# ServiceFoundation/partisan

Measured on AMD Instinct MI355X. Metric: simulated node-rounds/sec (+ msgs/sec), 1M-node HyParView+Plumtree, higher is better.
Workload: dtype u32

## Files before the change

### partisan_amd/csrc/psim_consume.hip

```cpp
#include "psim_device.h"
#include "psim_kernels.h"
#include "psim_lite.h"
#include "psim_wave.h"

namespace psim {

#define ID_OF(e, n) (((uint32_t)(e) << 20) | (uint32_t)(n))
#define ID_E(id) ((id) >> 20)
#define ID_C(id) ((id)&0xFFFFFu)

constexpr int WAVES_PER_BLOCK = 4;
#ifndef PSIM_WAVES_PER_SIMD
#define PSIM_WAVES_PER_SIMD 4
#endif

#ifdef PSIM_STAMPS
__device__ unsigned long long g_stamps[32];
__device__ unsigned long long g_stamps_lite[32];
#define STAMP(w, k)                                                                  \
    do {                                                                             \
        uint64_t t_ = __builtin_amdgcn_s_memtime();                                  \
        if (lane_id() == 0) (w).stl[(k)] += t_ - (w).t_last;                         \
        (w).t_last = t_;                                                             \
    } while (0)
// ... 1819 lines not shown
    uint4* o = reinterpret_cast<uint4*>(a.rec_out + slot);
    o[0] = make_uint4(dst, me, tt, seq);
    o[1] = make_uint4(a0, a1, a2, 0u);
    if (!PSIM_SHORT_TAIL || ((tt >> 16) & 0xFFu)) {
        o[2] = make_uint4(X[0], X[1], X[2], X[3]);
        o[3] = make_uint4(X[4], X[5], X[6], X[7]);
    }
    a.okey[slot] = dst | (max_emit(tt & 0xFF) << KEY_DST_BITS);
    return dg;
}

DEV void block_append(bool go, const uint4& D, uint4* desc, uint32_t* cnt, uint32_t* wcnt) {
    const uint64_t m = ballot(go);
    const uint32_t wv = threadIdx.x >> 6;
    __syncthreads();
    if (lane_id() == 0) wcnt[wv] = popc(m);
    __syncthreads();
    if (threadIdx.x == 0) {
        uint32_t t = 0;
        for (uint32_t k = 0; k < (blockDim.x >> 6); k++) t += wcnt[k];
        wcnt[4] = t ? atomicAdd(cnt, t) : 0u;
    }
    __syncthreads();
    if (go) {
        uint32_t b0 = wcnt[4];
        for (uint32_t k = 0; k < wv; k++) b0 += wcnt[k];
        desc[b0 + popc(m & lt_mask())] = D;
    }
}

#ifndef PSIM_RELAY_WAVES
#define PSIM_RELAY_WAVES 5
#endif
#ifndef PSIM_RELAY_FJ
#define PSIM_RELAY_FJ 1
#endif
#ifndef PSIM_PTL_BIN
#define PSIM_PTL_BIN 1
#endif
#ifndef PSIM_LITE_BIN
#define PSIM_LITE_BIN 1
#endif
__global__ void __launch_bounds__(256, PSIM_RELAY_WAVES) k_relay(RoundArgs) {
    if (*kargs().ctl) return;
    if (blockIdx.x == 0 && threadIdx.x == 0) kargs().ktime[0] = __builtin_amdgcn_s_memrealtime();
    enum { R_PROC, R_DELIV, R_SHUF, R_FAIL, R_DIGEST, R_BOUND, R_DELIV_FJ, R_FJ, R_N };
    __shared__ unsigned long long sst[R_N];
    __shared__ uint32_t wc5[11][5];
    if (threadIdx.x < R_N) sst[threadIdx.x] = 0;
    __syncthreads();
    const uint32_t l = lane_id();
    const uint32_t na = *kargs().n_alist;
    const uint64_t two58 = 1ull << 58;
    unsigned long long v[R_N] = {};
    for (uint32_t base = blockIdx.x * blockDim.x; base < na; base += gridDim.x * blockDim.x) {
        KArgs& a = kargs();
        const uint32_t P = base + threadIdx.x;
        uint4 D = make_uint4(0, 0, 0, 0);
        bool heavy = false, to_pt = false, relay = false, maps = false, shuf = false, lite = false, bcast = false, term = false,
             extra = false;
        Hdr h;
        uint32_t ik = 0, oend = 0;
        uint4 act0 = make_uint4(0, 0, 0, 0), act1 = act0;
        uint32_t me_part = 0;
        uint32_t hvm = 0;
        uint8_t fl0 = 0;
        if (P < na) {
            D = a.desc[P];
            const uint32_t id = D.x, tf = D.z >> 28;
            ik = D.z & DESC_CNT_MASK;
            const size_t li = id - a.lo;
            h = a.hdr[li];
            oend = (uint32_t)a.obase[li + 1];
            const uint4* ar = reinterpret_cast<const uint4*>(a.act + li * PSIM_ACTIVE_CAP);
            act0 = ar[0];
            act1 = ar[1];
            me_part = a.part[id];
            fl0 = a.flags[id];
            uint32_t hvn = 0;
            hvm = 0;
            bool all_relay = true, all_shuf = true, term_out = false, fjn = false;
            bcast = false; term = false; extra = (tf & DESC_SHUFFLE) != 0;
            const uint32_t av[8] = {act0.x, act0.y, act0.z, act0.w, act1.x, act1.y, act1.z, act1.w};
            for (uint32_t j = 0; j < ik; j += 4) {
                uint2 T[4];
#pragma unroll
                for (int q = 0; q < 4; q++) {
                    const uint4 r4 = j + q < ik ? *reinterpret_cast<const uint4*>(a.rec_in + D.y + j + q)
                                                : make_uint4(0, 0, (uint32_t)PSIM_MSG_PT_BROADCAST, 0);
                    T[q] = make_uint2(r4.y, r4.z);
                }
#pragma unroll
                for (int q = 0; q < 4; q++) {
                    const uint32_t tt = T[q].y, type = tt & 0xFF;
                    bcast |= j + q < ik && type == PSIM_MSG_PT_BROADCAST;
                    if (type < PSIM_MSG_PT_BROADCAST || type >= PSIM_MSG_XBOT_OPTIMIZATION) {
                        hvn++;
                        hvm |= j + q < 32 ? 1u << (j + q) : 0u;
                        maps |= type <= PSIM_MSG_NEIGHBOR_ACCEPTED;
                        const uint32_t ttl = (tt >> 8) & 0xFF;
                        const bool relays = ttl > 0 && h.act_n > 1;
                        const bool fj = PSIM_RELAY_FJ && !a.xbot && type == PSIM_MSG_FORWARD_JOIN && ttl > 0 &&
                                        ttl != a.prwl && h.act_n >= 4;
                        fjn |= fj;
                        all_relay &= (type == PSIM_MSG_SHUFFLE && ttl > 0) || fj;
                        all_shuf &= type == PSIM_MSG_SHUFFLE || type == PSIM_MSG_SHUFFLE_REPLY;
                        term |= type == PSIM_MSG_SHUFFLE && !relays;
                        extra |= type == PSIM_MSG_SHUFFLE && relays;
                        if (type == PSIM_MSG_SHUFFLE && !relays) {
                            bool in = false;
#pragma unroll
                            for (int k = 0; k < 8; k++) in |= (uint32_t)k < h.act_n && av[k] == T[q].x;
                            term_out |= !in;
                        }
                    }
                }
            }
            const bool fresh = h.start_round == a.round;
            bool exits = false;
            if (a.crash_round) {
                uint32_t cv[PSIM_CONN_CAP] = {};
                if (h.conn_n) {
                    const uint4* cr = reinterpret_cast<const uint4*>(a.conn + li * PSIM_CONN_CAP);
                    const uint4 c0 = cr[0], c1 = cr[1];
                    cv[0] = c0.x; cv[1] = c0.y; cv[2] = c0.z; cv[3] = c0.w;
                    cv[4] = c1.x; cv[5] = c1.y; cv[6] = c1.z; cv[7] = c1.w;
                }
#pragma unroll
                for (int j = 0; j < 8; j++) {
                    bool down = false;
#pragma unroll
                    for (int k = 0; k < PSIM_CONN_CAP; k++) down |= (uint32_t)k < h.conn_n && cv[k] == (av[j] | PSIM_CONN_DOWN);
                    exits |= (uint32_t)j < h.act_n && av[j] != id && av[j] < a.n_nodes && !down &&
                             crashed_now(a, av[j]);
                }
#pragma unroll
                for (int k = 0; k < PSIM_CONN_CAP; k++)
                    exits |= (uint32_t)k < h.conn_n && !(cv[k] & PSIM_CONN_DOWN) && crashed_now(a, cv[k] & KEY_DST_MASK);
            }
            const bool cdown = h.conn_dn != 0 && (hvn > 0 || (tf & DESC_SHUFFLE));
            const bool xwork = a.xbot && (h.conn_cl || (D.z & DESC_XBOT_BIT));
            bool fj_ok = true;
            if (fjn && a.plumtree) {
                const uint4* pr = reinterpret_cast<const uint4*>(a.pt_all + li * PSIM_PT_MEMBERS_CAP);
                const uint4 p0 = pr[0], p1 = pr[1];
                const uint32_t pv[8] = {p0.x, p0.y, p0.z, p0.w, p1.x, p1.y, p1.z, p1.w};
                fj_ok = h.all_n == h.act_n;
#pragma unroll
                for (int j = 0; j < 8; j++) {
                    bool in = false;
#pragma unroll
                    for (int k = 0; k < 8; k++) in |= (uint32_t)k < h.all_n && pv[k] == av[j];
                    fj_ok &= (uint32_t)j >= h.act_n || in;
                }
            }
            heavy = exits || fresh || ((tf & DESC_PROMO) && h.act_n < a.min_active) ||
                    (hvn && !all_shuf && !(all_relay && fj_ok)) || term_out || cdown || xwork;
            lite = !heavy && hvn && !(all_relay && h.act_n > 1);
            shuf = !heavy && !lite && (tf & DESC_SHUFFLE);
            maps = maps || exits || (tf & DESC_PROMO) || h.conn_cl;
            relay = !heavy && !lite && hvn > 0;
            const bool pt_msgs = !fresh && ik > hvn, origin = (tf & DESC_ORIGIN) != 0;
            const bool lazy = (tf & DESC_LAZY) && h.out_n > 0;
            to_pt = a.plumtree && (pt_msgs || origin || lazy);
            if (!heavy && !lite && (relay || to_pt || shuf)) v[R_PROC]++;
        }
        uint32_t upm[4] = {NONE, NONE, NONE, NONE};
        if (P < na && (relay || lite)) {
            const uint32_t av[8] = {act0.x, act0.y, act0.z, act0.w, act1.x, act1.y, act1.z, act1.w};
            KArgs& a = kargs();
#pragma unroll
            for (int j = 0; j < 8; j += 2) {
                const uint32_t q0 = (uint32_t)j < h.act_n && av[j] < a.n_nodes ? av[j] : D.x;
                const uint32_t q1 = (uint32_t)j + 1 < h.act_n && av[j + 1] < a.n_nodes ? av[j + 1] : D.x;
                upm[j >> 1] = (uint32_t)a.upart[q0] | ((uint32_t)a.upart[q1] << 16);
            }
        }
        const bool origin_node = ((D.z >> 28) & DESC_ORIGIN) != 0;
        {
            const bool ptl = P < na && to_pt && !origin_node, lt = P < na && lite;
            const bool pe = ptl && (!a.ptl_split || (!heavy && !lite && !shuf)), pl = ptl && !pe;
            const bool pb = bcast || !PSIM_PTL_BIN;
            const bool lt0 = lt && !(extra && PSIM_LITE_BIN), lt1 = lt && extra && PSIM_LITE_BIN;
            const bool tb = term || !PSIM_LITE_BIN;
            const bool g[11] = {P < na && heavy, P < na && to_pt && origin_node, pe && pb,
                                P < na && shuf, lt0 && tb, pe && !pb, lt0 && !tb,
                                lt1 && tb, lt1 && !tb, pl && pb, pl && !pb};
            uint64_t m[11];
#pragma unroll
            for (int k = 0; k < 11; k++) m[k] = ballot(g[k]);
            const uint32_t wv = threadIdx.x >> 6, nwv = blockDim.x >> 6;
            __syncthreads();
            if (l == 0)
#pragma unroll
                for (int k = 0; k < 11; k++) wc5[k][wv] = popc(m[k]);
            __syncthreads();
            if (threadIdx.x < 11) {
                const uint32_t k = threadIdx.x;
                uint32_t t = 0;
                for (uint32_t j = 0; j < nwv; j++) t += wc5[k][j];
                uint32_t* cnt = k == 0 ? a.n_slow : k == 1 ? a.n_pt : k == 2 ? a.n_ptl : k == 3 ? a.n_shuf
                              : k == 4 ? a.n_lite : k == 5 ? a.n_ptl + 1 : k < 9 ? a.n_lite + (k - 5)
                              : a.n_ptl + (k - 7);
                wc5[k][4] = t ? atomicAdd(cnt, t) : 0u;
            }
            __syncthreads();
#pragma unroll
            for (int k = 0; k < 11; k++)
                if (g[k]) {
                    uint32_t b0 = wc5[k][4];
                    for (uint32_t j = 0; j < wv; j++) b0 += wc5[k][j];
                    const uint32_t at = b0 + popc(m[k] & lt_mask());
                    uint4* desc = k == 0 ? a.desc_slow : k == 1 ? a.desc_pt : k == 2 || k == 5 || k >= 9 ? a.desc_ptl
                                : k == 3 ? a.desc_shuf : a.desc_lite;
                    const uint32_t nl = a.n_local;
                    desc[k == 5 || k == 6 ? nl - 1 - at : k == 7 || k == 9 ? nl + at
                         : k == 8 || k == 10 ? 2 * nl - 1 - at : at] =
                        k == 0 && maps ? make_uint4(D.x, D.y, D.z | DESC_MAPS_BIT, D.w) : D;
                }
        }
        if (P < na && lite && !heavy) {
            uint32_t cm = 0;
#pragma unroll
            for (int j = 0; j < 8; j++)
                cm |= ((upm[j >> 1] >> (16 * (j & 1))) & 0xFFFFu) == me_part ? 1u << j : 0u;
            kargs().lite_cm[D.x - kargs().lo] = (uint8_t)cm;
        }
        if (P >= na || heavy || lite) continue;
        const uint32_t id = D.x;
        const size_t li = id - a.lo;
        const uint32_t A[8] = {act0.x, act0.y, act0.z, act0.w, act1.x, act1.y, act1.z, act1.w};
        uint64_t rng = h.rng;
        uint32_t seq = 0;
        const bool big = ik > 32;
        uint32_t rm = relay ? hvm : 0u;
        for (uint32_t jr = 0; relay && (big ? jr < ik : rm != 0); jr++) {
            if (!big) {
                jr = (uint32_t)__ffs(rm) - 1;
                rm &= rm - 1;
            }
            const Msg* rp = a.rec_in + D.y + jr;
            const uint32_t tt = rp->tt;
            if ((tt & 0xFF) >= PSIM_MSG_PT_BROADCAST) continue;
            const bool fj = (tt & 0xFF) == PSIM_MSG_FORWARD_JOIN;
            const uint32_t ttl = (tt >> 8) & 0xFF, nex = (tt >> 16) & 0xFF, src = rp->src;
            const uint32_t jq = fj ? rp->a0 : NONE, jpe = fj ? rp->a1 : 0u;
            v[fj ? R_DELIV_FJ : R_DELIV]++;
            uint32_t elig = 0;
#pragma unroll
            for (int j = 0; j < 8; j++)
                elig |= (j < h.act_n && A[j] != src && A[j] != id && A[j] != jq) ? (1u << j) : 0u;
            const uint32_t cnt = __popc(elig);
            if (cnt) {
                uint32_t k;
                for (;;) {
                    const uint64_t x = draw58_at(rng++, id, a.seed);
                    if (x < cnt) { k = (uint32_t)x; break; }
                    const uint32_t i = mod_small(x, cnt);
                    if (x - i <= two58 - cnt) { k = i; break; }
                }
                uint32_t e = elig;
                for (uint32_t j = 0; j < k; j++) e &= e - 1;
                const uint32_t jr_ = (uint32_t)__ffs(e) - 1;
                const uint32_t r = A[jr_];
                uint32_t up = 0;
#pragma unroll
                for (int j = 0; j < 8; j++)
                    if ((uint32_t)j == jr_) up = (upm[j >> 1] >> (16 * (j & 1))) & 0xFFFFu;
                if (r < a.n_nodes && up == me_part) {
                    rng++;
                    uint32_t X[8] = {};
                    if (!fj) {
                        const uint4* ex = reinterpret_cast<const uint4*>(rp->ex);
                        const uint4 e0 = ex[0], e1 = ex[1];
                        const uint32_t E[8] = {e0.x, e0.y, e0.z, e0.w, e1.x, e1.y, e1.z, e1.w};
#pragma unroll
                        for (int j = 0; j < 8; j++) X[j] = (uint32_t)j < nex ? E[j] : 0u;
                    }
                    v[R_DIGEST] += relay_emit(a, D.w + seq, r, id,
                                              fj ? PSIM_MSG_FORWARD_JOIN | ((ttl - 1) << 8)
                                                 : PSIM_MSG_SHUFFLE | ((ttl - 1) << 8) | (nex << 16),
                                              seq, fj ? jq : 0u, jpe, 0u, X);
                    seq++;
                    v[fj ? R_FJ : R_SHUF]++;
                } else {
                    v[R_FAIL]++;
                }
            }
        }
        if (rng != h.rng) a.hdr[li].rng = rng;
        a.ocnt[li] = seq;
        v[R_BOUND] += seq > oend - D.w ? 1u : 0u;
        if (!to_pt) {
            a.flags[id] = (uint8_t)((fl0 & (F_UP | F_CRASHED)) | (h.out_n ? F_LAZY : 0) |
                                    (min((uint32_t)h.out_n, 15u) << F_OUTN_SHIFT) |
                                    (h.act_n < a.min_active ? F_LOWACT : 0));
        }
    }
#pragma unroll
    for (int k = 0; k < R_N; k++)
        for (int o = 32; o > 0; o >>= 1) v[k] += __shfl_xor(v[k], o);
    if (l == 0)
        for (int k = 0; k < R_N; k++)
            if (v[k]) atomicAdd(&sst[k], v[k]);
    __syncthreads();
    uint64_t* row = kargs().stat_relay + (size_t)blockIdx.x * NST;
    for (uint32_t k = threadIdx.x; k < NST; k += blockDim.x)
        row[k] = k == ST_PROC ? sst[R_PROC] : k == ST_DELIV + PSIM_MSG_SHUFFLE ? sst[R_DELIV]
               : k == ST_EMIT + PSIM_MSG_SHUFFLE ? sst[R_SHUF] : k == ST_FAIL ? sst[R_FAIL]
               : k == ST_DELIV + PSIM_MSG_FORWARD_JOIN ? sst[R_DELIV_FJ] : k == ST_EMIT + PSIM_MSG_FORWARD_JOIN ? sst[R_FJ]
               : k == ST_DIGEST ? sst[R_DIGEST] : k == ST_BOUND ? sst[R_BOUND] : 0ull;
}

constexpr int SHUF_TOPK = PSIM_EXCHANGE_CAP - 1;

DEV void topk_insert(uint64_t (&K)[SHUF_TOPK], uint32_t (&E)[SHUF_TOPK], uint64_t key, uint32_t e) {
    uint64_t ck = key;
    uint32_t ce = e;
#pragma unroll
    for (int i = 0; i < SHUF_TOPK; i++) {
        const bool lt = ck < K[i] || (ck == K[i] && ce < E[i]);
        const uint64_t tk = lt ? K[i] : ck;
        const uint32_t te = lt ? E[i] : ce;
        K[i] = lt ? ck : K[i];
        E[i] = lt ? ce : E[i];
        ck = tk;
        ce = te;
    }
}

enum { S_SHUF, S_FAIL, S_DIGEST, S_BOUND, S_N };
DEV void shuf_blocks(const uint32_t bid, const uint32_t nblk, unsigned long long* const sst) {
    if (*kargs().ctl) return;
    if (threadIdx.x < S_N) sst[threadIdx.x] = 0;
    __syncthreads();
    const uint32_t l = lane_id();
    const uint32_t ns = *kargs().n_shuf;
    const uint64_t two58 = 1ull << 58;
    unsigned long long v[S_N] = {};
    for (uint32_t P = bid * blockDim.x + threadIdx.x; P < ns; P += nblk * blockDim.x) {
        KArgs& a = kargs();
        const uint4 D = a.desc_shuf[P];
        const uint32_t id = D.x;
        const size_t li = id - a.lo;
        const uint64_t rng0 = a.hdr[li].rng;
        const uint32_t cnts = reinterpret_cast<const uint32_t*>(a.hdr + li)[9];
        const uint32_t act_n = cnts & 0xFF, pas_n = (cnts >> 8) & 0xFF;
        const uint4* ar = reinterpret_cast<const uint4*>(a.act + li * PSIM_ACTIVE_CAP);
        const uint4 a0 = ar[0], a1 = ar[1];
        const uint32_t A[8] = {a0.x, a0.y, a0.z, a0.w, a1.x, a1.y, a1.z, a1.w};
        uint32_t seq = a.ocnt[li];
        const uint32_t oend = (uint32_t)a.obase[li + 1];
        const uint32_t me_part = a.part[id];
        uint64_t rng = rng0;
        uint64_t K[SHUF_TOPK];
        uint32_t E[SHUF_TOPK];
#pragma unroll
// ... 762 lines not shown
```

### partisan_amd/csrc/psim_engine.hip

```cpp
#include <hip/hip_runtime.h>
#include <rccl/rccl.h>

#include <algorithm>
#include <chrono>
#include <cstdio>
#include <cstdlib>
#include <cstring>
#include <new>
#include <set>
#include <vector>

#include "psim_comm.h"
#include "psim_device.h"
#include "psim_kernels.h"
#include "psim_wave.h"

using namespace psim;

namespace {

constexpr int BLK = 256;
constexpr uint32_t PREP_BLK = 1024;
#ifndef PSIM_PREP_NPT
#define PSIM_PREP_NPT 4
// ... 1827 lines not shown
        release();
        p = nb.p; n = nb.n;
        return PSIM_OK;
    }
    int alloc(size_t want) {
        static const bool trace = getenv("PSIM_TRACE_GROW") != nullptr;
        if (trace && want >= (1u << 20)) std::fprintf(stderr, "psim: alloc %zu x %zu B\n", want, sizeof(T));
        if (hipMalloc(&p, std::max<size_t>(want, 1) * sizeof(T)) != hipSuccess) return PSIM_ENOMEM;
        n = want;
        if (hipMemset(p, 0, std::max<size_t>(want, 1) * sizeof(T)) != hipSuccess) return PSIM_EDEVICE;
        return PSIM_OK;
    }
    int alloc_on(size_t want, hipStream_t st) {
        if (hipMalloc(&p, std::max<size_t>(want, 1) * sizeof(T)) != hipSuccess) return PSIM_ENOMEM;
        n = want;
        if (hipMemsetAsync(p, 0, std::max<size_t>(want, 1) * sizeof(T), st) != hipSuccess) return PSIM_EDEVICE;
        return PSIM_OK;
    }
    void release() { if (p) (void)hipFree(p); p = nullptr; n = 0; }
};

template <typename T>
struct TmpBuf : DBuf<T> {
    TmpBuf() = default;
    TmpBuf(const TmpBuf&) = delete;
    TmpBuf& operator=(const TmpBuf&) = delete;
    ~TmpBuf() { this->release(); }
};

enum Kern { KT_EVENTS, KT_PREPARE, KT_CONSUME, KT_SCAN, KT_COMPACT, KT_SORT, KT_EXCHANGE, KT_GATHER,
            KT_STATS, KT_HOST_EXPORT, KT_HOST_IMPORT, KT_N };
const char* kKernName[KT_N] = {"events", "prepare", "consume", "scan", "compact", "sort",
                               "exchange", "gather", "stats", "k_host_export", "k_host_import"};

inline uint32_t grid_for(uint64_t n) { return (uint32_t)std::max<uint64_t>(1, (n + BLK - 1) / BLK); }

int bits_for(uint64_t n) {
    int b = 1;
    while (b < 32 && (1ull << b) < n) b++;
    return b;
}

constexpr uint64_t RESERVE_PER_NODE = 24;
constexpr uint64_t RCAP_PER_NODE = 4;
constexpr uint64_t RCAP_RESERVE = 8;
constexpr double RCAP_FREE_FRAC = 0.30;
constexpr double OUTBOX_SPARE = 0.12;

struct Shard {
    uint32_t idx = 0, lo = 0, n = 0;
    hipStream_t stream = nullptr;
    DBuf<uint8_t> flags, part;
    DBuf<upart_t> upart;
    DBuf<uint8_t> lite_cm;
    DBuf<uint32_t> crash_bits;
    DBuf<uint8_t> btab;
    DBuf<Hdr> hdr;
    DBuf<uint32_t> act, pas, pt_all, pt_com, pt_eag, pt_laz, pt_rt, start;
    DBuf<uint64_t> sentm, recvm, mapx;
    DBuf<uint32_t> mapx_top;
    DBuf<uint32_t> origin;
    DBuf<uint32_t> slots;
    DBuf<uint32_t> bc_roots, bc_msgs;
    DBuf<uint64_t> pt_out, outx;
    DBuf<uint32_t> conn;
    DBuf<uint32_t> outx_top;
    DBuf<uint32_t> ikeys, ivals;
    uint32_t m_in = 0;
    DBuf<Msg> outbox;
    DBuf<Wire> recvh, recvt;
    DBuf<uint32_t> wseg;
    std::vector<uint32_t> wseg_host;
    DBuf<Msg> inbox;
    DBuf<uint32_t> okey, ocnt, in_beg,
        d_nact, n_slow, n_pt, n_shuf, n_lite, n_ptl, rank, tmp, hist, hoff;
    DBuf<uint32_t> rtot, rbase;
    DBuf<uint32_t> gcnt;
    DBuf<unsigned long long> bmask;
    DBuf<uint2> pairs;
    DBuf<unsigned long long> cb;
    DBuf<unsigned long long> btot;
    DBuf<uint4> desc, desc_slow, desc_pt, desc_shuf, desc_lite, desc_ptl;
    DBuf<uint64_t> bound, pscan, obase, stat_part, stat_out, stat_tile, d_off;
    DBuf<uint8_t> cub_tmp;
    DBuf<uint32_t> ev_ids, ev_contacts, stop_ids, n_stop;
    bool tomb_live = false;
    DBuf<Wire> sendbuf;
    DBuf<uint32_t> sview, sinv, fbits, pay[2], pay_top;
    int pay_cur = 0;
    DBuf<uint8_t> faulted;
    DBuf<uint64_t> omit;
    std::vector<uint64_t> soff, scnt, lcnt;
    uint32_t pper = BLK;
    uint32_t pgrid = 0, cgrid = 0, rgrid = 0, tgrid = 0, sgrid = 0, lgrid = 0, qgrid = 0, egrid = 0;
    uint64_t* pin = nullptr;
    uint64_t* pin_dev = nullptr;
    static constexpr int MAXT = 32;
    hipEvent_t ev[MAXT][2];
    int tk[MAXT];
    int tn = 0;
    hipEvent_t wait_ev = nullptr;
    hipStream_t side[2] = {nullptr, nullptr};
    hipEvent_t fork_ev = nullptr, join_ev[2] = {nullptr, nullptr};
    bool ev_live = false;
    bool reserved = false;
    bool upart_valid = false;
    uint64_t rcap = 0;
// ... 30 lines not shown
    bool failed = false;
    std::vector<Shard*> shards;
    int rank = 0, world = 1;
    bool ranked = false;
    Comm* comm = nullptr;
    DBuf<uint64_t> comm_cnt;
    bool hosted = false, round_open = false;
    std::vector<Msg> host_out, host_in;
    std::vector<uint32_t> host_wbase;
    DBuf<Msg> hx_rec;
    DBuf<uint32_t> hx_wbase;
    PendingEvents open_ev;
    uint64_t x_records = 0, x_bytes = 0;
    std::vector<uint32_t> pend_crash, pend_join, pend_contact;
    std::vector<uint8_t> pend_join_mark;
    std::vector<uint32_t> pend_lv_a, pend_lv_t;
    std::vector<uint8_t> pend_part;
    bool pend_part_set = false, pend_part_clear = false;
    std::vector<uint32_t> pend_b_root, pend_b_msg;
    uint32_t slot_tab[2 * PSIM_MSG_SLOTS];
    uint32_t tracked_msg = PSIM_NONE;
    bool btab = false;
    uint32_t btab_hash = 0;
    uint32_t fw = 0;
    bool tomb = false;
    std::vector<uint8_t> started;
    std::set<uint64_t> nx_omit_s, nx_omit_r;
    std::vector<uint8_t> nx_faulted;
    size_t nx_nfaulted = 0;
    bool faults_dirty = false;
    uint32_t faults = 0, n_omit_s = 0, n_omit_r = 0;
    double kt_ms[KT_N] = {0};
    uint64_t kt_n[KT_N] = {0};
    bool phase_timers = false;
    uint32_t rb_blocks = RB_BLOCKS;
    uint32_t rr_reg = RR_REG;
    bool route_fused = true;
};

namespace {

inline bool local_route(const psim_handle* h) { return h->G == 1 && !h->ranked; }

constexpr int PTL_EARLY_DEFAULT = 0;
int ptl_early_knob() {
    static const int v = [] {
        const char* e = getenv("PSIM_PTL_EARLY");
        const int x = e && *e ? atoi(e) : -1;
        return x >= 0 && x <= 2 ? x : PTL_EARLY_DEFAULT;
    }();
    return v;
}

constexpr int PREP_FUSED_DEFAULT = 1;
bool prep_fused_knob() {
#ifdef PSIM_BOUND_TERMS
    return false;
#else
    static const bool v = [] {
        const char* e = getenv("PSIM_PREP_FUSED");
        return e && *e ? atoi(e) != 0 : PREP_FUSED_DEFAULT != 0;
    }();
    return v;
#endif
}

uint32_t route_wshift(uint32_t n) {
    uint32_t wshift = n > (1u << 26) ? 13 : n > (1u << 22) ? 12 : 11;
    static const int env = getenv("PSIM_ROUTE_WSHIFT") ? atoi(getenv("PSIM_ROUTE_WSHIFT")) : 0;
    if (env >= (int)WSHIFT_MIN && env <= (int)WSHIFT_MAX) wshift = (uint32_t)env;
    return wshift;
}

bool prep_fused_handle(const psim_handle* h, const Shard* s) {
    return prep_fused_knob() && h->G == 1 && !h->ranked && h->route_fused && s->n <= (1u << 26) &&
           h->cfg.manager != PSIM_MANAGER_PLUGGABLE;
}

RoundArgs make_args(psim_handle* h, Shard* s) {
    RoundArgs a;
    memset(&a, 0, sizeof a);
    const psim_config& c = h->cfg;
    a.n_nodes = h->N; a.round = (uint32_t)h->round; a.seed = c.seed;
    a.lo = s->lo; a.n_local = s->n;
    a.max_active = c.max_active_size; a.min_active = c.min_active_size;
    a.max_passive = c.max_passive_size; a.arwl = c.arwl; a.prwl = c.prwl;
    a.k_active = c.k_active; a.k_passive = c.k_passive;
    a.shuffle_period = c.shuffle_period; a.promotion_period = c.promotion_period;
    a.random_promotion = c.random_promotion; a.plumtree = c.plumtree;
    a.lazy_tick_period = c.lazy_tick_period;
    a.tracked_msg = h->tracked_msg;
    a.origin = s->origin.p;
    a.slots = s->slots.p;
    a.flags = s->flags.p; a.part = s->part.p; a.hdr = s->hdr.p; a.crash_bits = s->crash_bits.p;
    a.upart = s->upart.p;
    a.lite_cm = s->lite_cm.p;
    a.btab = h->btab ? s->btab.p : nullptr;
    a.act = s->act.p; a.pas = s->pas.p; a.sentm = s->sentm.p; a.recvm = s->recvm.p;
    a.mapx = s->mapx.p; a.mapx_top = s->mapx_top.p;
    a.mapx_rows = (uint32_t)(s->mapx.n / IDMAP_EXT);
    a.pt_all = s->pt_all.p; a.pt_com = s->pt_com.p; a.pt_eag = s->pt_eag.p; a.pt_laz = s->pt_laz.p;
    a.pt_rt = s->pt_rt.p;
    a.pt_out = s->pt_out.p; a.outx = s->outx.p; a.outx_top = s->outx_top.p;
    a.conn = s->conn.p;
    a.outx_rows = (uint32_t)(s->outx.n / OUT_EXT);
    a.start = s->start.p;
    a.pl = c.manager == PSIM_MANAGER_PLUGGABLE;
    a.xbot = c.manager == PSIM_MANAGER_XBOT; a.xbot_period = c.xbot_period;
    a.ptl_split = ptl_early_knob() != 0;
    a.strategy = c.strategy; a.periodic = c.periodic_interval; a.scamp_c = c.scamp_c;
    a.fanout = c.fanout; a.fw = h->fw; a.tomb = h->tomb;
    a.fbits = s->fbits.p; a.sview = s->sview.p; a.sinv = s->sinv.p;
    a.ktime = reinterpret_cast<unsigned long long*>(s->stat_out.p + NST);
    a.ctl = s->ctl.p;
    a.desc_slow = s->desc_slow.p; a.n_slow = s->n_slow.p;
    a.desc_pt = s->desc_pt.p; a.n_pt = s->n_pt.p;
    a.desc_shuf = s->desc_shuf.p; a.n_shuf = s->n_shuf.p;
    a.desc_lite = s->desc_lite.p; a.n_lite = s->n_lite.p;
    a.desc_ptl = s->desc_ptl.p; a.n_ptl = s->n_ptl.p;
    a.stop_ids = s->stop_ids.p; a.n_stop = s->n_stop.p;
    a.faults = h->faults; a.n_omit_s = h->n_omit_s; a.n_omit_r = h->n_omit_r;
    a.faulted = s->faulted.p; a.omit = s->omit.p;
    return a;
}

int route_buffers(Shard* s, bool both_inboxes);

struct KTimer {
    Shard* s;
    int slot;
    KTimer(psim_handle* h, Shard* s_, int k) : s(s_), slot(-1) {
        if (!h->phase_timers || s->tn >= Shard::MAXT) return;
        slot = s->tn++;
        s->tk[slot] = k;
        (void)hipEventRecord(s->ev[slot][0], s->stream);
    }
    ~KTimer() {
        if (slot >= 0) (void)hipEventRecord(s->ev[slot][1], s->stream);
    }
};

void flush_timers(psim_handle* h, Shard* s) {
    for (int i = 0; i < s->tn; i++) {
        float ms = 0;
        if (hipEventElapsedTime(&ms, s->ev[i][0], s->ev[i][1]) != hipSuccess) continue;
        h->kt_ms[s->tk[i]] += ms;
        h->kt_n[s->tk[i]]++;
    }
    s->tn = 0;
}

constexpr uint32_t SCAN_ITEMS = 8, SCAN_TILE = BLK * SCAN_ITEMS;

template <typename T, uint32_t NT>
__device__ T block_excl(T v, T* total) {
    __shared__ T wsum[NT / 64];
    const uint32_t l = threadIdx.x & 63, wv = threadIdx.x >> 6;
    T x = v;
#pragma unroll
    for (int d = 1; d < 64; d <<= 1) {
        const T y = __shfl_up(x, d);
        if (l >= (uint32_t)d) x += y;
// ... 2474 lines not shown
```

### partisan_amd/csrc/psim_kernels.h

```cpp
#pragma once
#include <stddef.h>

#include "psim_device.h"

namespace psim {

#ifndef PSIM_UPART8
#define PSIM_UPART8 1
#endif
#if PSIM_UPART8
typedef uint8_t upart_t;
#else
typedef uint16_t upart_t;
#endif

struct RoundArgs {
    uint32_t n_nodes, round;
    uint32_t lo, n_local;
    uint64_t seed;
    uint32_t max_active, min_active, max_passive, arwl, prwl, k_active, k_passive;
    uint32_t shuffle_period, promotion_period, random_promotion, plumtree, lazy_tick_period;
    uint32_t xbot, xbot_period;
    uint32_t ptl_split;
    uint32_t crash_round, tracked_msg;
    uint32_t upart_dirty;
    uint32_t lazy_wake;
    uint8_t* flags;
    const uint8_t* part;
    upart_t* upart;
    uint8_t* lite_cm;
    const uint32_t* crash_bits;
    const uint8_t* btab;
    Hdr* hdr;
    uint32_t *act, *pas;
    uint64_t *sentm, *recvm;
    uint64_t* mapx;
    uint32_t* mapx_top;
    uint32_t mapx_rows;
    uint32_t *pt_all, *pt_com, *pt_eag, *pt_laz, *pt_rt;
    uint32_t* conn;
    uint64_t* pt_out;
    uint64_t* outx;
    uint32_t* outx_top;
    uint32_t outx_rows;
    const uint32_t* origin;
    const uint32_t* slots;
    const uint32_t* in_beg;
    const unsigned long long* in_cb;
    const uint32_t* start;
    const uint4* desc;
    const uint32_t* n_alist;
    uint4* desc_slow;
    uint32_t* n_slow;
    uint4* desc_pt;
    uint32_t* n_pt;
    uint4* desc_shuf;
    uint32_t* n_shuf;
    uint64_t* stat_shuf;
    uint4* desc_lite;
    uint32_t* n_lite;
    uint64_t* stat_lite;
    uint4* desc_ptl;
    uint32_t* n_ptl;
    uint64_t* stat_ptl;
    uint64_t* stat_ptle;
    uint64_t* stat_relay;
    uint64_t* stat_pt;
    const Msg* rec_in;
    const uint64_t* obase;
    Msg* rec_out;
    uint32_t* okey;
    uint32_t* ocnt;
    uint64_t* stat_part;
    unsigned long long* ktime;
    const uint32_t* ctl;
    uint32_t pl, strategy, periodic, scamp_c, fanout;
    uint32_t fw;
    uint32_t tomb;
    uint32_t* fbits;
    const uint32_t* pay_in;
    uint32_t* pay_out;
    uint32_t* pay_top;
    uint32_t pay_cap;
// ... 40 lines not shown
uint32_t ptl_grid();

constexpr uint32_t CRASH_GRAIN_SHIFT = 4;
constexpr upart_t UPART_DOWN = (upart_t)(PSIM_UPART8 ? 0xFFu : 0x100u);
__device__ __forceinline__ bool crash_filter(const uint32_t* bits, uint32_t id) {
    const uint32_t g = id >> CRASH_GRAIN_SHIFT;
    return (bits[g >> 5] >> (g & 31)) & 1u;
}
template <class Args>
__device__ __forceinline__ bool crashed_now(Args& a, uint32_t id) {
    return crash_filter(a.crash_bits, id) && (a.flags[id] & F_CRASHED);
}

typedef const __attribute__((address_space(4))) RoundArgs KArgs;

template <class Args>
__device__ __forceinline__ uint4 ptl_desc(Args& a, const uint32_t (&c)[4], uint32_t i) {
    const uint32_t n = a.n_local;
    return a.desc_ptl[i < c[0] ? i
                    : i < c[0] + c[1] ? n - 1 - (i - c[0])
                    : i < c[0] + c[1] + c[2] ? n + (i - c[0] - c[1])
                    : 2 * n - 1 - (i - c[0] - c[1] - c[2])];
}
template <class Args>
__device__ __forceinline__ void ptl_counts(Args& a, uint32_t part, uint32_t (&c)[4], uint32_t& nq) {
    c[0] = part != PTL_LATE ? a.n_ptl[0] : 0u; c[1] = part != PTL_LATE ? a.n_ptl[1] : 0u;
    c[2] = part != PTL_EARLY ? a.n_ptl[2] : 0u; c[3] = part != PTL_EARLY ? a.n_ptl[3] : 0u;
    nq = c[0] + c[1] + c[2] + c[3];
}
template <class Args>
__device__ __forceinline__ uint32_t lite_at(Args& a, const uint32_t (&c)[4], uint32_t i) {
    const uint32_t n = a.n_local;
    return i < c[0] ? i
         : i < c[0] + c[1] ? n - 1 - (i - c[0])
         : i < c[0] + c[1] + c[2] ? n + (i - c[0] - c[1])
         : 2 * n - 1 - (i - c[0] - c[1] - c[2]);
}
template <class Args>
__device__ __forceinline__ void lite_counts(Args& a, uint32_t (&c)[4], uint32_t& na) {
    c[0] = a.n_lite[0]; c[1] = a.n_lite[1]; c[2] = a.n_lite[2]; c[3] = a.n_lite[3];
    na = c[0] + c[1] + c[2] + c[3];
}
#ifndef PSIM_SHORT_TAIL
#define PSIM_SHORT_TAIL 1
#endif

constexpr uint32_t layout_mix(uint32_t h, uint64_t v) {
    return ((h ^ (uint32_t)v) * 0x01000193u ^ (uint32_t)(v >> 32)) * 0x01000193u;
}
constexpr uint32_t layout_sig() {
    uint32_t h = 0x811C9DC5u;
    const uint64_t v[] = {
        PSIM_ABI_VERSION, sizeof(RoundArgs), offsetof(RoundArgs, flags), offsetof(RoundArgs, upart),
        offsetof(RoundArgs, hdr), offsetof(RoundArgs, conn), offsetof(RoundArgs, outx_rows),
        offsetof(RoundArgs, desc), offsetof(RoundArgs, desc_lite), offsetof(RoundArgs, stat_ptle), offsetof(RoundArgs, stat_pt),
        offsetof(RoundArgs, rec_out), offsetof(RoundArgs, okey), offsetof(RoundArgs, ktime),
        offsetof(RoundArgs, ctl), offsetof(RoundArgs, fbits), offsetof(RoundArgs, omit),
        sizeof(Hdr), sizeof(Msg), sizeof(upart_t), PSIM_SHORT_TAIL, PTL_BLOCK, KEY_DST_BITS, KEY_BCAST,
        PSIM_ACTIVE_CAP, PSIM_PASSIVE_CAP, PSIM_EXCHANGE_CAP, PSIM_PT_ROOTS, PSIM_PT_OUT_CAP, PSIM_IDMAP_CAP,
        PSIM_CONN_CAP, PSIM_SVIEW_CAP, OUT_IN, IDMAP_IN, RT_SET, RT_WORDS, NST, CRASH_GRAIN_SHIFT};
    for (uint64_t x : v) h = layout_mix(h, x);
    return h;
}
uint32_t layout_sig_consume();
uint32_t layout_sig_lite();
uint32_t layout_sig_strategy();

inline uint32_t resident_grid(const void* kernel, uint32_t block) {
    int dev = 0, nb = 0;
    hipDeviceProp_t p;
    if (hipGetDevice(&dev) != hipSuccess || hipGetDeviceProperties(&p, dev) != hipSuccess ||
        hipOccupancyMaxActiveBlocksPerMultiprocessor(&nb, kernel, (int)block, 0) != hipSuccess || nb <= 0)
        return 1024;
    return (uint32_t)nb * (uint32_t)p.multiProcessorCount;
}

__device__ __forceinline__ KArgs& kargs() {
    KArgs* p = (KArgs*)__builtin_amdgcn_kernarg_segment_ptr();
    asm volatile("" : "+s"(p));
    return *p;
}

}
```

### partisan_amd/csrc/psim_lite.h

```cpp
#pragma once
#include <utility>

#include "psim_device.h"
#include "psim_kernels.h"
#include "psim_wave.h"

namespace psim {
namespace lite {
namespace {

#ifndef PSIM_HALF_WPB
#define PSIM_HALF_WPB 4
#endif
#ifndef PSIM_HALF_WAVES
#define PSIM_HALF_WAVES 4
#endif
#ifndef PSIM_QUARTER_WPB
#define PSIM_QUARTER_WPB 4
#endif
#ifndef PSIM_QUARTER_WAVES
#define PSIM_QUARTER_WAVES 4
#endif
#ifndef PSIM_QUARTER_STAGE
#define PSIM_QUARTER_STAGE 8
// ... 482 lines not shown
}

template <uint32_t W>
struct In {
    uint4 D;
    uint32_t r0, r1, w9, A, part;
    typename Pas<W>::Row P;
    uint32_t cm, oe;
    uint32_t SRC, TT;
    uint32_t EXP;
};

DEV uint4 load_desc(KArgs& a, const uint32_t (&lc)[4], uint32_t i, bool live) {
    return live ? a.desc_lite[lite_at(a, lc, i)] : make_uint4(0, 0, 0, 0);
}
template <uint32_t W>
DEV void load_rows(KArgs& a, In<W>& in, bool live) {
    const uint32_t l = Grp<W>::lane();
    const size_t li = live ? in.D.x - a.lo : 0;
    const uint32_t* hrow = reinterpret_cast<const uint32_t*>(a.hdr + li);
    in.r0 = hrow[0]; in.r1 = hrow[1]; in.w9 = hrow[9];
    in.A = l < PSIM_ACTIVE_CAP ? a.act[li * PSIM_ACTIVE_CAP + l] : 0u;
    in.P = Pas<W>::load(a.pas + li * PSIM_PASSIVE_CAP);
    in.part = a.part[live ? in.D.x : 0];
    in.cm = a.lite_cm[li];
    in.oe = reinterpret_cast<const uint32_t*>(a.obase + li + 1)[0];
}
template <uint32_t W>
DEV In<W> load_in(KArgs& a, const uint4& D) {
    const uint32_t l = Grp<W>::lane();
    In<W> in;
    in.D = D;
    in.r0 = in.r1 = in.w9 = in.A = in.part = in.cm = in.oe = 0;
    in.P = {};
    const uint32_t ik = in.D.z & DESC_CNT_MASK;
    const Msg* r = a.rec_in + in.D.y + (l < ik ? l : 0u);
    const uint2 st = *reinterpret_cast<const uint2*>(&r->src);
    in.SRC = l < ik ? st.x : 0u;
    in.TT = l < ik ? st.y : (uint32_t)PSIM_MSG_PT_BROADCAST;
    in.EXP = a.rec_in[in.D.y + ((l >> 3) < ik ? (l >> 3) : 0u)].ex[l & 7];
    return in;
}

template <uint32_t W>
DEV void begin(Node<W>& x, const In<W>& in) {
    const uint32_t l = Grp<W>::lane();
    x.me = in.D.x; x.ib = in.D.y;
    x.ik = in.D.z & DESC_CNT_MASK; x.ob = in.D.w;
    x.fl = (in.D.z >> 28) | (in.part << 8) | (in.w9 & 0xFFFF0000u);
    x.rng = ((uint64_t)in.r1 << 32) | in.r0;
    x.act_n = in.w9 & 0xFF; x.pas_n = (in.w9 >> 8) & 0xFF;
    x.A = l < x.act_n ? in.A : 0u;
    x.pas.set(in.P, x.pas_n);
    x.seq = 0; x.flushed = 0;
    x.dcb = ~0ull;
}

template <uint32_t W>
DEV void body(Node<W>& x, Lds<W>& w, Cnt& c, const In<W>& in) {
    using G = Grp<W>;
    KArgs& a = kargs();
    const uint32_t l = G::lane();
    for (uint32_t cb = 0; cb < x.ik; cb += W) {
      uint32_t SRC = in.SRC, TT = in.TT;
      if (cb) {
          const bool has = cb + l < x.ik;
          const uint2 st = *reinterpret_cast<const uint2*>(&a.rec_in[x.ib + (has ? cb + l : 0u)].src);
          SRC = has ? st.x : 0u;
          TT = has ? st.y : (uint32_t)PSIM_MSG_PT_BROADCAST;
      }
      uint32_t M = G::mask((TT & 0xFF) < PSIM_MSG_PT_BROADCAST);
      while (M) {
        const uint32_t j = (uint32_t)__ffs(M) - 1;
        M &= M - 1;
        const uint32_t p = G::get(SRC, j), tt = G::get(TT, j);
        const uint32_t ep = G::get(in.EXP, (j << 3) | (l & 7));
        const uint32_t q = cb + j;
        uint32_t ex = q < G::PREF ? ep : a.rec_in[x.ib + q].ex[l & 7];
        const uint32_t nex = (tt >> 16) & 0xFF, ttl = (tt >> 8) & 0xFF;
        const uint32_t type = tt & 0xFF;
        ex = l < nex ? ex : 0u;
        const bool reply = type == PSIM_MSG_SHUFFLE_REPLY;
        const bool relay = !reply && ttl > 0 && x.act_n > 1;
        c.dl += reply ? 0x10000u : 1u;
        LSTAMP(w, 6);
        if (relay) {
            const uint32_t r = select_random(x, w, x.A, x.act_n, p, x.me);
            if (r != PSIM_NONE) hv_send(x, w, c, r, PSIM_MSG_SHUFFLE, ttl - 1, ex, nex);
            LSTAMP(w, 1);
        } else {
            if (!reply) {
                uint32_t RESP = 0;
                const uint32_t nr = Pas<W>::sublist(x, w, nex, RESP, 0);
                LSTAMP(w, 2);
                hv_send(x, w, c, p, PSIM_MSG_SHUFFLE_REPLY, 0, RESP, nr);
                LSTAMP(w, 3);
            }
            merge_exchange(x, w, ex, nex, !reply);
            LSTAMP(w, 4);
        }
      }
    }
    if (x.fl & DESC_SHUFFLE) {
        uint32_t EX = l == 0 ? x.me : 0u;
        uint32_t m = 1;
        m = sublist<PSIM_ACTIVE_CAP>(x, w, x.A, x.act_n, a.k_active, EX, m);
        m = Pas<W>::sublist(x, w, a.k_passive, EX, m);
// ... 40 lines not shown
    using G = Grp<W>;
    static constexpr uint32_t SREC = (NST * 2 + 3) & ~3u, SKEY = SREC + G::WPB * G::N * G::STAGE * 16,
                              SCR = SKEY + G::WPB * G::N * G::STAGE, WORDS = SCR + G::WPB * G::N * G::SCR;
};
template <uint32_t W>
DEV void lite_kernel(const uint32_t bid, const uint32_t nblk, uint32_t* const pool) {
    using G = Grp<W>;
    constexpr uint32_t WPB = G::WPB, STAGE = G::STAGE;
    static_assert(STAGE >= 1 && STAGE <= 16, "flush writes a group's staged route keys one per lane");
    static_assert((STAGE * 16 * 4) % 16 == 0, "a group's staging area is read in 16-B pieces");
    static_assert(sizeof(Msg) == 16 * 4, "a record is one word per lane of a group's first row");
    static_assert(PSIM_PASSIVE_CAP == 32, "the passive row is one entry a lane of a half, two a lane of a row");
    static_assert(PSIM_ACTIVE_CAP <= 8 && PSIM_EXCHANGE_CAP == 8,
                  "a record's exchange ids move from lanes 0-7 to lanes 8-15 (row_shr:8)");
    static_assert(G::SCR >= PSIM_PASSIVE_CAP, "a sublist scatters one word per passive entry");
    static_assert(WPB * G::N * (STAGE * 16 + STAGE + G::SCR) * 4 + NST * 8 <= 64 * 1024,
                  "the block's LDS: four blocks of it per CU at 4 waves/SIMD");
    if (*kargs().ctl) return;
    unsigned long long* const sst = reinterpret_cast<unsigned long long*>(pool);
    uint32_t* const srecs = pool + Carve<W>::SREC;
    uint32_t* const skeys = pool + Carve<W>::SKEY;
    uint32_t* const scrs = pool + Carve<W>::SCR;
#ifdef PSIM_STAMPS
    __shared__ unsigned long long stls[WPB][32];
    for (int i = threadIdx.x; i < (int)(WPB * 32); i += blockDim.x) (&stls[0][0])[i] = 0;
#endif
    for (int i = threadIdx.x; i < NST; i += blockDim.x) sst[i] = 0;
    __syncthreads();
    const uint32_t wid = threadIdx.x >> 6, g = G::idx();
    Lds<W> w;
    w.sst = sst;
    w.srec = srecs + (wid * G::N + g) * (STAGE * 16);
    w.skey = skeys + (wid * G::N + g) * STAGE;
    w.scr = scrs + (wid * G::N + g) * G::SCR;
    w.KM = G::magic_lanes();
#ifdef PSIM_STAMPS
    w.stl = stls[wid];
    w.t_last = __builtin_amdgcn_s_memtime();
#endif
    Cnt c = {};
    const uint32_t nw = nblk * WPB;
    const uint32_t first = G::N * (bid * WPB + wid) + g;
    const uint32_t step = G::N * nw;
    uint32_t lc[4], na;
    lite_counts(kargs(), lc, na);
    if (first < na) {
        Node<W> x;
        In<W> in = load_in<W>(kargs(), load_desc(kargs(), lc, first, true));
        load_rows(kargs(), in, true);
        uint4 Dn = load_desc(kargs(), lc, first + step < na ? first + step : first, first + step < na);
        for (uint32_t i = first; i < na; i += step) {
            LSTAMP(w, 8);
            begin(x, in);
            x.AF = in.cm | (min(in.oe - x.ob, 0xFFFFFFu) << 8);
            const uint32_t nx = i + step, nnx = i + 2 * step;
            In<W> inn = load_in<W>(kargs(), Dn);
            LSTAMP(w, 0);
            body(x, w, c, in);
            LSTAMP(w, 9);
            Dn = load_desc(kargs(), lc, nnx < na ? nnx : i, nnx < na);
            load_rows(kargs(), inn, nx < na);
            writeback(x, w, c);
            LSTAMP(w, 7);
            in = inn;
        }
        count(w, c);
    }
    {
        uint64_t dg = c.digest;
#pragma unroll
        for (int off = 32; off > 0; off >>= 1) dg += __shfl_xor(dg, off);
        if (__lane_id() == 0 && dg) atomicAdd(&sst[ST_DIGEST], (unsigned long long)dg);
    }
    __syncthreads();
    for (int i = threadIdx.x; i < NST; i += blockDim.x)
        kargs().stat_lite[(size_t)bid * NST + i] = sst[i];
#ifdef PSIM_STAMPS
    if (threadIdx.x < 32) {
        unsigned long long t = 0;
        for (uint32_t k = 0; k < WPB; k++) t += stls[k][threadIdx.x];
        if (t) atomicAdd(&g_stamps_half[threadIdx.x], t);
    }
#endif
}

}
}
}
```

Measured before the change: 2.974 billion.

## Pre-relay leading shuffle messages for lite nodes in relay kernel

For lite nodes, the relay kernel now handles the leading run of relaying SHUFFLE messages itself. It records the emitted sequence count in a widened 16-bit lite_cm entry and advances the descriptor past those messages, so the lite kernel starts later in the inbox and seeds its output sequence from the stored count. This moves simple relay work out of the heavier lite path and hoists the partition-match mask computation so it is computed once per node. It also reworks the stat counters to 32-bit with a separate 64-bit digest accumulator reduced via ds_bpermute, and adds a PSIM_RELAY_LEAD knob that is on by default. The risk is that the relay kernel takes on more divergent work, and descriptor offsets must stay consistent across kernels.

```diff
diff --git a/partisan_amd/csrc/psim_consume.hip b/partisan_amd/csrc/psim_consume.hip
--- a/partisan_amd/csrc/psim_consume.hip
+++ b/partisan_amd/csrc/psim_consume.hip
@@ -1895,7 +1895,8 @@
     const uint32_t l = lane_id();
     const uint32_t na = *kargs().n_alist;
     const uint64_t two58 = 1ull << 58;
-    unsigned long long v[R_N] = {};
+    uint32_t v[R_N] = {};
+    unsigned long long vdg = 0;
     for (uint32_t base = blockIdx.x * blockDim.x; base < na; base += gridDim.x * blockDim.x) {
         KArgs& a = kargs();
         const uint32_t P = base + threadIdx.x;
@@ -1907,6 +1908,7 @@
         uint4 act0 = make_uint4(0, 0, 0, 0), act1 = act0;
         uint32_t me_part = 0;
         uint32_t hvm = 0;
+        uint32_t first = 0;
         uint8_t fl0 = 0;
         if (P < na) {
             D = a.desc[P];
@@ -1923,6 +1925,7 @@
             uint32_t hvn = 0;
             hvm = 0;
             bool all_relay = true, all_shuf = true, term_out = false, fjn = false;
+            uint32_t nf = ~0u;
             bcast = false; term = false; extra = (tf & DESC_SHUFFLE) != 0;
             const uint32_t av[8] = {act0.x, act0.y, act0.z, act0.w, act1.x, act1.y, act1.z, act1.w};
             for (uint32_t j = 0; j < ik; j += 4) {
@@ -1950,6 +1953,7 @@
                         all_shuf &= type == PSIM_MSG_SHUFFLE || type == PSIM_MSG_SHUFFLE_REPLY;
                         term |= type == PSIM_MSG_SHUFFLE && !relays;
                         extra |= type == PSIM_MSG_SHUFFLE && relays;
+                        nf = type == PSIM_MSG_SHUFFLE && relays ? nf : min(nf, j + q);
                         if (type == PSIM_MSG_SHUFFLE && !relays) {
                             bool in = false;
 #pragma unroll
@@ -2000,6 +2004,7 @@
             heavy = exits || fresh || ((tf & DESC_PROMO) && h.act_n < a.min_active) ||
                     (hvn && !all_shuf && !(all_relay && fj_ok)) || term_out || cdown || xwork;
             lite = !heavy && hvn && !(all_relay && h.act_n > 1);
+            first = a.relay_lead && lite && ik <= 32 && nf < ik ? nf : 0u;
             shuf = !heavy && !lite && (tf & DESC_SHUFFLE);
             maps = maps || exits || (tf & DESC_PROMO) || h.conn_cl;
             relay = !heavy && !lite && hvn > 0;
@@ -2059,25 +2064,23 @@
                     const uint32_t nl = a.n_local;
                     desc[k == 5 || k == 6 ? nl - 1 - at : k == 7 || k == 9 ? nl + at
                          : k == 8 || k == 10 ? 2 * nl - 1 - at : at] =
-                        k == 0 && maps ? make_uint4(D.x, D.y, D.z | DESC_MAPS_BIT, D.w) : D;
+                        k == 0 && maps ? make_uint4(D.x, D.y, D.z | DESC_MAPS_BIT, D.w)
+                        : k == 4 || (k >= 6 && k <= 8) ? make_uint4(D.x, D.y + first, D.z - first, D.w) : D;
                 }
         }
-        if (P < na && lite && !heavy) {
-            uint32_t cm = 0;
-#pragma unroll
-            for (int j = 0; j < 8; j++)
-                cm |= ((upm[j >> 1] >> (16 * (j & 1))) & 0xFFFFu) == me_part ? 1u << j : 0u;
-            kargs().lite_cm[D.x - kargs().lo] = (uint8_t)cm;
-        }
-        if (P >= na || heavy || lite) continue;
+        if (P >= na || heavy) continue;
         const uint32_t id = D.x;
         const size_t li = id - a.lo;
         const uint32_t A[8] = {act0.x, act0.y, act0.z, act0.w, act1.x, act1.y, act1.z, act1.w};
         uint64_t rng = h.rng;
         uint32_t seq = 0;
+        uint32_t cm = 0;
+#pragma unroll
+        for (int j = 0; j < 8; j++)
+            cm |= ((upm[j >> 1] >> (16 * (j & 1))) & 0xFFFFu) == me_part ? 1u << j : 0u;
         const bool big = ik > 32;
-        uint32_t rm = relay ? hvm : 0u;
-        for (uint32_t jr = 0; relay && (big ? jr < ik : rm != 0); jr++) {
+        uint32_t rm = relay ? hvm : hvm & ((1u << first) - 1u);
+        for (uint32_t jr = 0; big ? relay && jr < ik : rm != 0; jr++) {
             if (!big) {
                 jr = (uint32_t)__ffs(rm) - 1;
                 rm &= rm - 1;
@@ -2088,7 +2091,8 @@
             const bool fj = (tt & 0xFF) == PSIM_MSG_FORWARD_JOIN;
             const uint32_t ttl = (tt >> 8) & 0xFF, nex = (tt >> 16) & 0xFF, src = rp->src;
             const uint32_t jq = fj ? rp->a0 : NONE, jpe = fj ? rp->a1 : 0u;
-            v[fj ? R_DELIV_FJ : R_DELIV]++;
+            v[R_DELIV] += fj ? 0u : 1u;
+            v[R_DELIV_FJ] += fj ? 1u : 0u;
             uint32_t elig = 0;
 #pragma unroll
             for (int j = 0; j < 8; j++)
@@ -2106,11 +2110,7 @@
                 for (uint32_t j = 0; j < k; j++) e &= e - 1;
                 const uint32_t jr_ = (uint32_t)__ffs(e) - 1;
                 const uint32_t r = A[jr_];
-                uint32_t up = 0;
-#pragma unroll
-                for (int j = 0; j < 8; j++)
-                    if ((uint32_t)j == jr_) up = (upm[j >> 1] >> (16 * (j & 1))) & 0xFFFFu;
-                if (r < a.n_nodes && up == me_part) {
+                if (r < a.n_nodes && ((cm >> jr_) & 1u)) {
                     rng++;
                     uint32_t X[8] = {};
                     if (!fj) {
@@ -2120,18 +2120,23 @@
 #pragma unroll
                         for (int j = 0; j < 8; j++) X[j] = (uint32_t)j < nex ? E[j] : 0u;
                     }
-                    v[R_DIGEST] += relay_emit(a, D.w + seq, r, id,
+                    vdg += relay_emit(a, D.w + seq, r, id,
                                               fj ? PSIM_MSG_FORWARD_JOIN | ((ttl - 1) << 8)
                                                  : PSIM_MSG_SHUFFLE | ((ttl - 1) << 8) | (nex << 16),
                                               seq, fj ? jq : 0u, jpe, 0u, X);
                     seq++;
-                    v[fj ? R_FJ : R_SHUF]++;
+                    v[R_SHUF] += fj ? 0u : 1u;
+                    v[R_FJ] += fj ? 1u : 0u;
                 } else {
                     v[R_FAIL]++;
                 }
             }
         }
         if (rng != h.rng) a.hdr[li].rng = rng;
+        if (lite) {
+            a.lite_cm[li] = (uint16_t)(cm | (seq << 8));
+            continue;
+        }
         a.ocnt[li] = seq;
         v[R_BOUND] += seq > oend - D.w ? 1u : 0u;
         if (!to_pt) {
@@ -2141,11 +2146,16 @@
         }
     }
 #pragma unroll
-    for (int k = 0; k < R_N; k++)
-        for (int o = 32; o > 0; o >>= 1) v[k] += __shfl_xor(v[k], o);
-    if (l == 0)
-        for (int k = 0; k < R_N; k++)
-            if (v[k]) atomicAdd(&sst[k], v[k]);
+    for (int k = 0; k < R_N; k++) {
+        unsigned long long t = k == R_DIGEST ? vdg : (unsigned long long)v[k];
+        for (uint32_t o = 32; o > 0; o >>= 1) {
+            const int from = (int)(((threadIdx.x & 63u) ^ o) << 2);
+            const uint32_t lo = (uint32_t)__builtin_amdgcn_ds_bpermute(from, (int)(uint32_t)t);
+            const uint32_t hi = (uint32_t)__builtin_amdgcn_ds_bpermute(from, (int)(uint32_t)(t >> 32));
+            t += ((unsigned long long)hi << 32) | lo;
+        }
+        if ((threadIdx.x & 63u) == 0 && t) atomicAdd(&sst[k], t);
+    }
     __syncthreads();
     uint64_t* row = kargs().stat_relay + (size_t)blockIdx.x * NST;
     for (uint32_t k = threadIdx.x; k < NST; k += blockDim.x)
diff --git a/partisan_amd/csrc/psim_engine.hip b/partisan_amd/csrc/psim_engine.hip
--- a/partisan_amd/csrc/psim_engine.hip
+++ b/partisan_amd/csrc/psim_engine.hip
@@ -1903,7 +1903,7 @@
     hipStream_t stream = nullptr;
     DBuf<uint8_t> flags, part;
     DBuf<upart_t> upart;
-    DBuf<uint8_t> lite_cm;
+    DBuf<uint16_t> lite_cm;
     DBuf<uint32_t> crash_bits;
     DBuf<uint8_t> btab;
     DBuf<Hdr> hdr;
@@ -2040,6 +2040,15 @@
     return v;
 }
 
+constexpr int RELAY_LEAD_DEFAULT = 1;
+bool relay_lead_knob() {
+    static const bool v = [] {
+        const char* e = getenv("PSIM_RELAY_LEAD");
+        return e && *e ? atoi(e) != 0 : RELAY_LEAD_DEFAULT != 0;
+    }();
+    return v;
+}
+
 constexpr int PREP_FUSED_DEFAULT = 1;
 bool prep_fused_knob() {
 #ifdef PSIM_BOUND_TERMS
@@ -2096,6 +2105,7 @@
     a.pl = c.manager == PSIM_MANAGER_PLUGGABLE;
     a.xbot = c.manager == PSIM_MANAGER_XBOT; a.xbot_period = c.xbot_period;
     a.ptl_split = ptl_early_knob() != 0;
+    a.relay_lead = relay_lead_knob() && h->lite.kernel != psim::k_consume_lite;
     a.strategy = c.strategy; a.periodic = c.periodic_interval; a.scamp_c = c.scamp_c;
     a.fanout = c.fanout; a.fw = h->fw; a.tomb = h->tomb;
     a.fbits = s->fbits.p; a.sview = s->sview.p; a.sinv = s->sinv.p;
diff --git a/partisan_amd/csrc/psim_kernels.h b/partisan_amd/csrc/psim_kernels.h
--- a/partisan_amd/csrc/psim_kernels.h
+++ b/partisan_amd/csrc/psim_kernels.h
@@ -22,13 +22,14 @@
     uint32_t shuffle_period, promotion_period, random_promotion, plumtree, lazy_tick_period;
     uint32_t xbot, xbot_period;
     uint32_t ptl_split;
+    uint32_t relay_lead;
     uint32_t crash_round, tracked_msg;
     uint32_t upart_dirty;
     uint32_t lazy_wake;
     uint8_t* flags;
     const uint8_t* part;
     upart_t* upart;
-    uint8_t* lite_cm;
+    uint16_t* lite_cm;
     const uint32_t* crash_bits;
     const uint8_t* btab;
     Hdr* hdr;
@@ -175,6 +176,7 @@
     uint32_t h = 0x811C9DC5u;
     const uint64_t v[] = {
         PSIM_ABI_VERSION, sizeof(RoundArgs), offsetof(RoundArgs, flags), offsetof(RoundArgs, upart),
+        offsetof(RoundArgs, relay_lead), sizeof(*RoundArgs().lite_cm),
         offsetof(RoundArgs, hdr), offsetof(RoundArgs, conn), offsetof(RoundArgs, outx_rows),
         offsetof(RoundArgs, desc), offsetof(RoundArgs, desc_lite), offsetof(RoundArgs, stat_ptle), offsetof(RoundArgs, stat_pt),
         offsetof(RoundArgs, rec_out), offsetof(RoundArgs, okey), offsetof(RoundArgs, ktime),
diff --git a/partisan_amd/csrc/psim_lite.h b/partisan_amd/csrc/psim_lite.h
--- a/partisan_amd/csrc/psim_lite.h
+++ b/partisan_amd/csrc/psim_lite.h
@@ -558,7 +558,7 @@
     x.act_n = in.w9 & 0xFF; x.pas_n = (in.w9 >> 8) & 0xFF;
     x.A = l < x.act_n ? in.A : 0u;
     x.pas.set(in.P, x.pas_n);
-    x.seq = 0; x.flushed = 0;
+    x.seq = in.cm >> 8; x.flushed = x.seq;
     x.dcb = ~0ull;
 }
 
@@ -705,7 +705,7 @@
         for (uint32_t i = first; i < na; i += step) {
             LSTAMP(w, 8);
             begin(x, in);
-            x.AF = in.cm | (min(in.oe - x.ob, 0xFFFFFFu) << 8);
+            x.AF = (in.cm & 0xFFu) | (min(in.oe - x.ob, 0xFFFFFFu) << 8);
             const uint32_t nx = i + step, nnx = i + 2 * step;
             In<W> inn = load_in<W>(kargs(), Dn);
             LSTAMP(w, 0);
```

Measured after the change: 3.103 billion (median of 6 runs). 1.04x the previous value.
